# HyeonwooNoh/VQA-Transfer-ExternalData

Measured on AMD Instinct MI355X. Metric: VQA train samples/sec (img+question) at bs512, higher is better.
Workload: dtype f32

## Files before the change

include/vqa_hot.h:

```cpp
#ifndef VQA_HOT_H
#define VQA_HOT_H

#include <stdint.h>

#ifdef __cplusplus
extern "C" {
#endif

#define VQA_HOT_ABI_VERSION 5

enum {
    VQA_OK = 0,
    VQA_ERR_ARG = -1,
    VQA_ERR_ALIGN = -2,
    VQA_ERR_LAUNCH = -3,
    VQA_ERR_UNSUPPORTED = -4,
    VQA_ERR_WORKSPACE = -5
};

int vqa_hot_version(void);
const char* vqa_hot_error_string(int code);

int vqa_gather_features(const float* table, const int32_t* nbox_table, const int64_t* idx,
                        float* V, int32_t* nb, int B, int R, int D, int64_t N, void* stream);
// ... 145 lines not shown
int vqa_vtail_supported(int rep, int R, int H, int D);
int vqa_vtail_set_mode(int mode);
int vqa_attn_pool_bwd_ds(const float* dpooled, const float* V, const float* att, float* ds, float* part_db, int B, int rep,
                         int R, int H, int D, void* stream);
int vqa_attn_pool_bwd_ds_v16(const float* dpooled, const uint16_t* V, const float* att, float* ds, float* part_db, int B,
                             int rep, int R, int H, int D, void* stream);
int vqa_ln_relu_att_bwd(const float* ds, const float* qv, const float* w, const uint8_t* keep_att, float keep_prob,
                        const float* pre, const float* mean, const float* rstd, const float* gamma, const float* beta,
                        float* dpre, float* part_dgamma, float* part_dbeta, float* part_dbias, float* dqv, float* part_dw,
                        int B, int rep, int R, int H, int D, void* stream);
int64_t vqa_colsum_vtail_workspace_floats(int M, int N);
int vqa_colsum_vtail(const float* X0, const float* X1, const float* X2, const float* X3, const float* Xb, int M, int N,
                     float* out0, float* out1, float* out2, float* out3, float* outb, float* workspace,
                     int64_t workspace_floats, void* stream);

enum {
    VQA_STAT_LOSS_TRAIN = 0, VQA_STAT_LOSS_REPORT, VQA_STAT_ALL_SCORE, VQA_STAT_EXIST_SCORE,
    VQA_STAT_TEST_SCORE, VQA_STAT_TEST_OBJ_SCORE, VQA_STAT_TEST_ATTR_SCORE, VQA_STAT_TRAIN_EXIST_SCORE,
    VQA_STAT_MAX_EXIST, VQA_STAT_MAX_TRAIN_EXIST, VQA_STAT_TEST_OBJ_MAX, VQA_STAT_TEST_ATTR_MAX,
    VQA_STAT_TEST_MAX, VQA_STAT_TEST_MAX_EXIST, VQA_STAT_MAX_TRAIN, VQA_STAT_COUNT = 16
};
int vqa_loss_fwd(const float* z, const float* target, const float* train_mask, const float* obj_mask,
                 const float* attr_mask, const float* exist_mask, int use_train_mask_in_loss, float inv_batch,
                 float* stats, int32_t* pred, float* dz, int B, int A, void* stream);
int vqa_loss2_fwd(const float* z_fixed, const float* z_tuned, const float* target, const float* train_mask,
                  const float* obj_mask, const float* attr_mask, const float* exist_mask, float inv_batch, float* stats,
                  int32_t* pred, float* dz_fixed, float* dz_tuned, float* z_sum, int sum_mode, int B, int A, void* stream);
int vqa_rowmin_mask_fwd(const float* z, const float* exist_mask, float* z_masked, float* rowmin, int B, int A, void* stream);
int vqa_rowmin_mask_bwd(float* dz, const float* z, const float* rowmin, const float* exist_mask, int B, int A, void* stream);
int vqa_softmax_ce_fwd(const float* z, const int32_t* label, const float* valid, int topk,
// ... 36 lines not shown
                                 const float* bias, uint64_t seed, uint64_t offset, float keep_prob, float* att, float* pooled,
                                 int B, int rep, int R, int H, int D, void* stream);
int vqa_attn_pool_bwd_rep_seeded(const float* dpooled, const float* v, const float* qv, const float* V, const float* att,
                                 const float* w, uint64_t seed, uint64_t offset, float keep_prob, float* dv, float* dqv,
                                 float* part_dw, float* part_db, int B, int rep, int R, int H, int D, void* stream);
int vqa_ln_act_fwd_seeded(const float* pre, const float* gamma, const float* beta, uint64_t seed, uint64_t offset,
                          float keep_prob, float* y, float* mean, float* rstd, int G, int rows, int N, int act, void* stream);
int vqa_ln_act_bwd_seeded(const float* dy, const float* pre, const float* mean, const float* rstd, const float* gamma,
                          const float* beta, uint64_t seed, uint64_t offset, float keep_prob, float* dpre,
                          float* part_dgamma, float* part_dbeta, float* part_dbias, int G, int rows, int N, int act,
                          void* stream);
int vqa_ln_relu_att_bwd_seeded(const float* ds, const float* qv, const float* w, uint64_t seed, uint64_t offset,
                               float keep_prob, const float* pre, const float* mean, const float* rstd, const float* gamma,
                               const float* beta, float* dpre, float* part_dgamma, float* part_dbeta, float* part_dbias,
                               float* dqv, float* part_dw, int B, int rep, int R, int H, int D, void* stream);

typedef struct {
    int32_t B, R, D, H, T, W, A, Vq;
    int64_t N_img;
    int32_t model_type;
    float keep_att;
    float keep_joint;
    float inv_global_batch;
    int32_t flags;
    int32_t num_marginal;
    int32_t ent_cols;
    float extra_weight;
    int32_t map_dim;
    int32_t La;
} vqa_dims_t;
// ... 74 lines not shown
    int32_t keep_seeded;
} vqa_batch_t;
#define VQA_KEEP_SITE_ATT 1
#define VQA_KEEP_SITE_JOINT 2
#define VQA_KEEP_SITE_JOINT2 4
#define VQA_KEEP_SITE_TILE 8
#define VQA_KEEP_SITE_WORD 16

int64_t vqa_fusion_workspace_bytes(const vqa_dims_t* dims);
int vqa_fusion_tensor(const vqa_dims_t* dims, const char* name, int64_t* offset_bytes, int64_t* n_elems);
int vqa_fusion_forward(const vqa_dims_t* dims, const vqa_params_t* params, const vqa_batch_t* batch,
                       void* workspace, int64_t workspace_bytes, int want_dz, void* stream);
int vqa_fusion_backward(const vqa_dims_t* dims, const vqa_params_t* params, const vqa_params_t* grads,
                        const vqa_batch_t* batch, void* workspace, int64_t workspace_bytes,
                        float* embed_slice_sq, void* stream);

typedef struct {
    int32_t B, n, R, D, H, W, A, Vq, n_ws;
    int32_t L;
    int32_t flags;
    float keep_att, keep_joint;
    float global_valid[2];
} vqa_pretrain_dims_t;

typedef struct { float *w, *b, *beta[4], *gamma[4]; } vqa_pt_fc_t;

typedef struct {
    float* wordset_map;
    float* l_glove;
    vqa_pt_fc_t spat_v_linear_v;
// ... 302 lines not shown
```

vqa-transfer-externaldata_amd/_lib.py:

```python
from __future__ import annotations

import ctypes as C
import os

_HERE = os.path.dirname(os.path.abspath(__file__))
_LIB_PATH = os.path.join(_HERE, "libvqahot.so")


class VqaHotError(RuntimeError):
    pass


def lib_path():
    return _LIB_PATH


class Dims(C.Structure):
    _fields_ = [("B", C.c_int32), ("R", C.c_int32), ("D", C.c_int32), ("H", C.c_int32), ("T", C.c_int32),
                ("W", C.c_int32), ("A", C.c_int32), ("Vq", C.c_int32), ("N_img", C.c_int64),
                ("model_type", C.c_int32), ("keep_att", C.c_float), ("keep_joint", C.c_float),
                ("inv_global_batch", C.c_float), ("flags", C.c_int32),
                ("num_marginal", C.c_int32), ("ent_cols", C.c_int32), ("extra_weight", C.c_float),
                ("map_dim", C.c_int32), ("La", C.c_int32)]

# ... 212 lines not shown
    "vqa_attn_pool_fwd_rep": (_I, [_P, _P, _P, _P, _P, _P, _P, _F, _P, _P, _I, _I, _I, _I, _I, _P]),
    "vqa_attn_pool_bwd_rep": (_I, [_P, _P, _P, _P, _P, _P, _P, _F, _P, _P, _P, _P, _I, _I, _I, _I, _I, _P]),
    "vqa_vtail_supported": (_I, [_I, _I, _I, _I]),
    "vqa_vtail_set_mode": (_I, [_I]),
    "vqa_gru_h0skip_set_mode": (_I, [_I]),
    "vqa_attn_pool_bwd_ds": (_I, [_P, _P, _P, _P, _P, _I, _I, _I, _I, _I, _P]),
    "vqa_attn_pool_bwd_ds_v16": (_I, [_P, _P, _P, _P, _P, _I, _I, _I, _I, _I, _P]),
    "vqa_ln_relu_att_bwd": (_I, [_P, _P, _P, _P, _F] + [_P] * 11 + [_I, _I, _I, _I, _I, _P]),
    "vqa_attn_pool_fwd_seeded": (_I, [_P, _P, _P, _I, _P, _P, _P, _U, _U, _F, _P, _P, _I, _I, _I, _I, _I, _P]),
    "vqa_attn_pool_bwd_seeded": (_I, [_P, _P, _P, _P, _I, _P, _P, _U, _U, _F, _P, _P, _P, _P, _I, _I, _I, _I, _I, _P]),
    "vqa_attn_pool_fwd_rep_seeded": (_I, [_P, _P, _P, _P, _P, _P, _U, _U, _F, _P, _P, _I, _I, _I, _I, _I, _P]),
    "vqa_attn_pool_bwd_rep_seeded": (_I, [_P, _P, _P, _P, _P, _P, _U, _U, _F, _P, _P, _P, _P, _I, _I, _I, _I, _I, _P]),
    "vqa_ln_act_fwd_seeded": (_I, [_P, _P, _P, _U, _U, _F, _P, _P, _P, _I, _I, _I, _I, _P]),
    "vqa_ln_act_bwd_seeded": (_I, [_P, _P, _P, _P, _P, _P, _U, _U, _F, _P, _P, _P, _P, _I, _I, _I, _I, _P]),
    "vqa_ln_relu_att_bwd_seeded": (_I, [_P, _P, _P, _U, _U, _F] + [_P] * 11 + [_I, _I, _I, _I, _I, _P]),
    "vqa_colsum_vtail_workspace_floats": (_L, [_I, _I]),
    "vqa_colsum_vtail": (_I, [_P] * 5 + [_I, _I] + [_P] * 6 + [_L, _P]),
    "vqa_loss_fwd": (_I, [_P, _P, _P, _P, _P, _P, _I, _F, _P, _P, _P, _I, _I, _P]),
    "vqa_loss2_fwd": (_I, [_P, _P, _P, _P, _P, _P, _P, _F, _P, _P, _P, _P, _P, _I, _I, _I, _P]),
    "vqa_rowmin_mask_fwd": (_I, [_P, _P, _P, _P, _I, _I, _P]),
    "vqa_rowmin_mask_bwd": (_I, [_P, _P, _P, _P, _I, _I, _P]),
    "vqa_report_reduce": (_I, [_P, _I, _P, _P]),
    "vqa_report_key": (C.c_char_p, [_I]),
    "vqa_sumsq": (_I, [_P, _L, _P, _P, _P, _L, _P]),
    "vqa_sumsq_workspace_floats": (_L, [_L]),
    "vqa_clip_adam": (_I, [_P, _P, _P, _P, _L, _P, _F, _F, _F, _F, _F, _P]),
    "vqa_dropout_mask": (_I, [_P, _L, C.c_uint64, C.c_uint64, _F, _P]),
    "vqa_clip_adam_dev": (_I, [_P, _P, _P, _P, _L, _P, _F, _P, _F, _F, _F, _P]),
    "vqa_embed2_fwd": (_I, [_P, _P, _P, _P, _I, _I, _I, _I, _P]),
    "vqa_embed2_bwd": (_I, [_P, _P, _P, _P, _I, _I, _I, _I, _P]),
# ... 139 lines not shown
```

vqa-transfer-externaldata_amd/csrc/attention.hip:

```cpp
#include "keep_launch.h"

namespace {

constexpr int MAX_R = 1024;

typedef float f32x4v __attribute__((ext_vector_type(4)));
typedef unsigned u32x2v __attribute__((ext_vector_type(2)));

template <typename VT> struct VMem;
template <> struct VMem<float> {
    typedef f32x4v Raw;
    static __device__ __forceinline__ Raw load(const float* __restrict__ p, int64_t i4) { return reinterpret_cast<const f32x4v*>(p)[i4]; }
    static __device__ __forceinline__ f32x4v widen(Raw r) { return r; }
    static __device__ __forceinline__ float4 load_f4(const float* __restrict__ p, int64_t i4) { return reinterpret_cast<const float4*>(p)[i4]; }
};
template <> struct VMem<uint16_t> {
    typedef u32x2v Raw;
    static __device__ __forceinline__ Raw load(const uint16_t* __restrict__ p, int64_t i4) { return reinterpret_cast<const u32x2v*>(p)[i4]; }
    static __device__ __forceinline__ f32x4v widen(Raw r) {
        f32x4v x;
        x.x = __uint_as_float(r.x << 16); x.y = __uint_as_float(r.x & 0xFFFF0000u);
        x.z = __uint_as_float(r.y << 16); x.w = __uint_as_float(r.y & 0xFFFF0000u);
        return x;
    }
// ... 119 lines not shown
        for (int k = 0; k < H4L; ++k) {
            const f32x4v q = qw4[lane + 64 * k];
            if (KP != KEEP_NONE) {
                const unsigned mm = m[i][k];
                acc += (x[i][k].x * q.x * (float)(mm & 0xFFu) + x[i][k].y * q.y * (float)((mm >> 8) & 0xFFu) +
                        x[i][k].z * q.z * (float)((mm >> 16) & 0xFFu) + x[i][k].w * q.w * (float)(mm >> 24)) * inv_keep;
            } else {
                acc += x[i][k].x * q.x + x[i][k].y * q.y + x[i][k].z * q.z + x[i][k].w * q.w;
            }
        }
        acc = wave_sum(acc);
        if (lane == 0 && row0 + 8 * i < R) s[row0 + 8 * i] = acc + bias0;
    }
}

template <int H4L, int D4T, int KP, typename VT = float, typename... KS>
__global__ __launch_bounds__(FWD_THREADS, 4) void attn_pool_fwd_fast_kernel(
    const float* __restrict__ v, const float* __restrict__ qv, const VT* __restrict__ V,
    const int32_t* __restrict__ nb, const float* __restrict__ w, const float* __restrict__ bias,
    const uint8_t* __restrict__ keepmask, float inv_keep, float* __restrict__ att_out, float* __restrict__ pooled, int R,
    int rep, KS... ks) {
    constexpr int H = H4L * 256, D = D4T * 2048, D4 = D / 4;
    extern __shared__ __attribute__((aligned(16))) float lds[];
    float* qw = lds;
    float* s = lds + H;
    const int b = blockIdx.x, lane = threadIdx.x & 63, wave = threadIdx.x >> 6;
    const int mem = b / rep;
    const f32x4v* vb4 = reinterpret_cast<const f32x4v*>(v + (int64_t)mem * R * H);
    const unsigned* mb4 = KP == KEEP_BYTES ? reinterpret_cast<const unsigned*>(keepmask + (int64_t)b * R * H) : nullptr;
    const VT* Vb = V + (int64_t)mem * R * D;

    typename VMem<VT>::Raw xv[FAST_PF][D4T];
#pragma unroll
    for (int j = 0; j < FAST_PF; ++j)
#pragma unroll
        for (int c = 0; c < D4T; ++c) xv[j][c] = VMem<VT>::load(Vb, (int64_t)min(j, R - 1) * D4 + threadIdx.x + c * FWD_THREADS);

    for (int h = threadIdx.x; h < H; h += FWD_THREADS) qw[h] = qv[(int64_t)b * H + h] * w[h];
    const float bias0 = bias[0];

    const f32x4v* qw4 = reinterpret_cast<const f32x4v*>(qw);
    if constexpr (KP == KEEP_SEEDED) {
        KeepSeed sq = keep_seed_of(ks...);
        sq.word0 += (uint64_t)b * R * (H / 4);
        attn_score_rows<H4L, 3, KP>(vb4, mb4, qw4, s, R, wave, inv_keep, bias0, lane, true, sq);
        attn_score_rows<H4L, 2, KP>(vb4, mb4, qw4, s, R, wave + 24, inv_keep, bias0, lane, false, sq);
    } else {
        attn_score_rows<H4L, 3, KP>(vb4, mb4, qw4, s, R, wave, inv_keep, bias0, lane, true);
        attn_score_rows<H4L, 2, KP>(vb4, mb4, qw4, s, R, wave + 24, inv_keep, bias0, lane, false);
    }
    __syncthreads();

    if (wave == 0) {
        const int n_valid = nb[mem];
        float mx = -INFINITY;
        for (int r = lane; r < R; r += 64) {
            const float x = (r < n_valid) ? s[r] : -INFINITY;
// ... 821 lines not shown
    VQA_CHECK_LAUNCH();
    return VQA_OK;
}

extern "C" int vqa_attn_pool_bwd_ds_v16(const float* dpooled, const uint16_t* V, const float* att, float* ds, float* part_db,
                                        int B, int rep, int R, int H, int D, void* stream) {
    VQA_REQUIRE(dpooled && V && att && ds && part_db && B >= 0, VQA_ERR_ARG);
    VQA_REQUIRE(vqa_vtail_supported(rep, R, H, D), VQA_ERR_UNSUPPORTED);
    VQA_REQUIRE(vqa_aligned16(dpooled) && v_aligned(V), VQA_ERR_ALIGN);
    if (B == 0) return VQA_OK;
    hipLaunchKernelGGL(attn_pool_bwd_ds_kernel<uint16_t>, dim3(B), dim3(BWD_THREADS), 0, (hipStream_t)stream, dpooled, V, att,
                       ds, part_db, R);
    VQA_CHECK_LAUNCH();
    return VQA_OK;
}
```

vqa-transfer-externaldata_amd/csrc/fusion_model.hip:

```cpp
#include <stdlib.h>
#include <string.h>

#include <string>
#include <vector>

#include "keep_launch.h"

namespace {

struct Entry { const char* name; int64_t off; int64_t n; int esz; };

struct Layout {
    std::vector<Entry> e;
    int64_t total = 0;
    int64_t add(const char* name, int64_t n, int esz = 4) {
        const int64_t off = total;
        e.push_back({name, off, n, esz});
        total += ((n * esz + 255) / 256) * 256;
        return off;
    }
    const Entry* find(const char* name) const {
        for (const auto& x : e)
            if (strcmp(x.name, name) == 0) return &x;
        return nullptr;
// ... 167 lines not shown

inline bool env_on(const char* name, bool dflt) {
    const char* e = getenv(name);
    return e == nullptr ? dflt : atoi(e) != 0;
}
inline bool xcat_enabled() { static const bool v = env_on("VQA_HOT_XCAT", true); return v; }
inline bool repack_enabled() { static const bool v = env_on("VQA_HOT_REPACK", false); return v; }
inline bool gru_ws_on() { static const bool v = env_on("VQA_HOT_GRU_WS", true); return v; }
inline bool visual_late_enabled() { static const bool v = env_on("VQA_HOT_VISUAL_LATE", true); return v; }
inline bool ln_pair_enabled() { static const bool v = env_on("VQA_HOT_LN_PAIR", true); return v; }
int g_vtail_mode = -1;
inline int vtail_mode() {
    if (g_vtail_mode < 0) g_vtail_mode = env_on("VQA_HOT_VTAIL", true) ? 1 : 0;
    return g_vtail_mode;
}
int g_h0skip_mode = -1;
inline int h0skip_mode() {
    if (g_h0skip_mode < 0) {
        const char* e = getenv("VQA_HOT_GRU_H0SKIP");
        g_h0skip_mode = e == nullptr ? 1 : (atoi(e) & 3);
    }
    return g_h0skip_mode;
}
int side_max_blocks() {
    static int v = -1;
    if (v < 0) {
        const char* e = getenv("VQA_HOT_SIDE_BLOCKS");
        v = e ? atoi(e) : 0;
    }
    return v;
// ... 381 lines not shown
        if (n_elems) *n_elems = (int64_t)dims->B * dims->H;
        return VQA_OK;
    }
    const Entry* e = L.find(key);
    if (e == nullptr) return VQA_ERR_ARG;
    if (offset_bytes) *offset_bytes = e->off;
    if (n_elems) *n_elems = e->n;
    return VQA_OK;
}

extern "C" int vqa_vtail_set_mode(int mode) {
    g_vtail_mode = mode < 0 ? -1 : (mode ? 1 : 0);
    return vtail_mode();
}

extern "C" int vqa_gru_h0skip_set_mode(int mode) {
    g_h0skip_mode = mode < 0 ? -1 : (mode & 3);
    return h0skip_mode();
}

namespace {

struct Step {
    const vqa_dims_t& d;
    const vqa_params_t* const P;
    const vqa_params_t* const G;
    const vqa_batch_t* const bt;
    const Layout L;
    const Ctx c;
    const int mt;
// ... 43 lines not shown
    const bool ws_ok = gru_ws_on() && (live_rows == nullptr || (T > 0 && live_rows[T - 1] > 0));
    if (ws_ok && (dir == GRU_FWD ? vqa_gru_ws_supported((int)T, (int)B, (int)H) : vqa_gru_ws_bwd_supported((int)T, (int)B, (int)H)) == 1)
        return GRU_WS;
    return live_rows != nullptr ? GRU_LIVE : GRU_CHAINS;
}


void fwd_visual_plan(Step& s) {
    s.sd = &side_stream();
    s.forked = fork_side(s.c, *s.sd);
    s.fuse_gather = !(s.d.flags & VQA_FLAG_BF16_GEMM) && gather_mode(&s.d) == 1 && (s.D % 32 == 0) && (s.H % 4 == 0) &&
                    vqa_aligned16(s.bt->table);
    s.visual_late = !s.forked && visual_late_enabled();
}

int fwd_visual(const Step& s) {
    const Ctx cv = s.side_ctx();
    const vqa_params_t* P = s.P;
    const vqa_batch_t* bt = s.bt;
    const int64_t B = s.B, R = s.R, D = s.D, H = s.H;
    {
        ProbeScope ps("gather", cv.st);
        if (feat16(s.d))
            TRY(vqa_gather_features_bf16(reinterpret_cast<const uint16_t*>(bt->table), bt->nbox_table, bt->image_idx,
                                         cv.u16("V_ft"), cv.i32("num_V_ft"), (int)B, (int)R, (int)D, s.d.N_img, cv.st));
        else
            TRY(vqa_gather_features(bt->table, bt->nbox_table, bt->image_idx, s.fuse_gather ? nullptr : cv.f("V_ft"),
                                    cv.i32("num_V_ft"), (int)B, (int)R, (int)D, s.d.N_img, cv.st));
    }
    if (s.fuse_gather) {
        {
            ProbeScope ps("v_linear_v.fwd_gemm", cv.st);
            TRY(vqa_gemm_f32_gather((int)(B * R), (int)H, (int)D, bt->table, (int)D, bt->image_idx, (int)R, s.d.N_img,
                                    P->v_linear_v.w, (int)H, cv.f("pre_v"), (int)H, P->v_linear_v.b, cv.f("V_ft"), (int)D,
                                    cv.st));
        }
        ProbeScope ps("v_linear_v.ln_fwd", cv.st);
        TRY(vqa_ln_relu_fwd(cv.f("pre_v"), P->v_linear_v.gamma, P->v_linear_v.beta, nullptr, 1.f, cv.f("v_linear_v"),
                            cv.f("mean_v"), cv.f("rstd_v"), (int)B, (int)R, (int)H, cv.st));
    } else {
        TRY(fc_ln_relu_fwd(cv, cv.f("V_ft"), B * R, D, H, P->v_linear_v, (int)R, "pre_v", "v_linear_v", "mean_v", "rstd_v",
                           NO_KEEP, 1.f));
    }
    if (s.mt == VQA_MODEL_ADAPT) {
        VQA_REQUIRE(P->v_adapt.w != nullptr && P->v_adapt.gamma != nullptr, VQA_ERR_ARG);
        TRY(fc_ln_relu_fwd(cv, cv.f("V_ft"), B * R, D, H, P->v_adapt, (int)R, "pre_va", "v_adapt", "mean_va", "rstd_va",
                           NO_KEEP, 1.f));
    }
    return VQA_OK;
}

int fwd_question(Step& s) {
    const Ctx& c = s.c;
    const vqa_params_t* P = s.P;
    const vqa_batch_t* bt = s.bt;
    const int64_t B = s.B, H = s.H, T = s.T, W = s.W, Wp = s.Wp;
    if (s.mt == VQA_MODEL_BI) {
        TRY(bi_question_fwd(c, P, bt));
// ... 72 lines not shown
                                (int)B, (int)H, c.st));
            s.lin_in = c.f("q_L_mean_noise");
        }
    }
    return VQA_OK;
}

int fwd_q_linear_v(const Step& s) {
    return fc_ln_relu_fwd(s.c, s.qv_in, s.B, s.H, s.H, s.P->q_linear_v, 1, "pre_qv", "q_linear_v", "mean_qv", "rstd_qv", NO_KEEP, 1.f);
}

int fwd_attention(const Step& s) {
    const Ctx& c = s.c;
    ProbeScope ps("attn_pool.fwd", c.st);
    const bool v16 = feat16(s.d);
    const void* V = v16 ? (const void*)c.u16("V_ft") : (const void*)c.f(s.mt == VQA_MODEL_ADAPT ? "v_adapt" : "V_ft");
    return vqa_attn_fwd_run(c.f("v_linear_v"), c.f("q_linear_v"), V, v16, c.i32("num_V_ft"), s.P->score.w, s.P->score.b,
                            keep_site(s.bt, VQA_KEEP_SITE_ATT).src(s.d.keep_att, s.H), c.f("att_score"), c.f("pooled_V_ft"),
                            (int)s.B, 1, (int)s.R, (int)s.H, (int)s.Dp, c.st);
}

int fwd_linear_l(Step& s) {
    const Ctx& c = s.c;
    const vqa_params_t* P = s.P;
    const int64_t B = s.B, H = s.H, Dp = s.Dp;
    s.pair = ln_pair_ok(s.d, P);
    if (!s.pair) {
        TRY(fc_ln_relu_fwd(c, c.f("pooled_V_ft"), B, Dp, H, P->pooled_linear_l, 1, "pre_pl", "pooled_linear_l", "mean_pl",
                           "rstd_pl", NO_KEEP, 1.f));
        return fc_ln_relu_fwd(c, s.lin_in, B, H, H, P->q_linear_l, 1, "pre_ll", "l_linear_l", "mean_ll", "rstd_ll", NO_KEEP, 1.f);
// ... 108 lines not shown
    fwd_visual_plan(s);
    if (!s.visual_late) TRY(fwd_visual(s));
    TRY(side_record(s));
    TRY(fwd_question(s));
    TRY(fwd_question_code(s));
    TRY(fwd_q_linear_v(s));
    TRY(side_wait(s));
    if (s.visual_late) TRY(fwd_visual(s));
    TRY(fwd_attention(s));
    TRY(fwd_linear_l(s));
    TRY(fwd_joint(s));
    TRY(fwd_head(s));
    return fwd_loss(s, want_dz);
}

extern "C" int vqa_fusion_backward(const vqa_dims_t* dims, const vqa_params_t* P, const vqa_params_t* G,
                                   const vqa_batch_t* bt, void* workspace, int64_t workspace_bytes,
                                   float* embed_slice_sq, void* stream) {
    return vqa_fusion_backward_phases(dims, P, G, bt, workspace, workspace_bytes, embed_slice_sq, 15, stream);
}

namespace {


int bwd_head(const Step& s) {
    const Ctx& c = s.c;
    const vqa_params_t* P = s.P;
    const vqa_params_t* G = s.G;
    const int64_t B = s.B, H = s.H, W = s.W, A = s.A;
    ProbeScope ps_head("head.bwd_gemm", c.st);
// ... 172 lines not shown
                                         (int)R, (int)H, (int)D, c.st));
        }
        {
            ProbeScope ps("v_linear_v.ln_bwd", c.st);
            TRY(vqa_ln_relu_att_bwd_run(c.f("ds"), c.f("q_linear_v"), P->score.w, keep_site(bt, VQA_KEEP_SITE_ATT).src(s.d.keep_att, H),
                                        c.f("pre_v"), c.f("mean_v"), c.f("rstd_v"), P->v_linear_v.gamma, P->v_linear_v.beta,
                                        c.f("d_pre_v"), c.part(0), c.part(1), c.part(2), c.f("d_qv"), c.f("part_dw"), (int)B, 1, (int)R,
                                        (int)H, (int)D, c.st));
            TRY(vqa_colsum_vtail(c.part(0), c.part(1), c.part(2), c.f("part_dw"), c.f("part_db"), (int)B, (int)H,
                                 G->v_linear_v.gamma, G->v_linear_v.beta, G->v_linear_v.b, G->score.w, G->score.b, c.colsum_ws(),
                                 c.colsum_ws_floats(), c.st));
        }
        ProbeScope ps("v_linear_v.dw_gemm", c.st);
        return gemm_x(c, 1, D, H, B * R, c.f("V_ft"), (int)D, c.f("d_pre_v"), (int)H, G->v_linear_v.w, (int)H);
    }
    {
        ProbeScope ps("attn_pool.bwd", c.st);
        const bool v16 = feat16(s.d);
        const void* V = v16 ? (const void*)c.u16("V_ft") : (const void*)c.f(s.mt == VQA_MODEL_ADAPT ? "v_adapt" : "V_ft");
        TRY(vqa_attn_bwd_run(c.f("d_pooled"), c.f("v_linear_v"), c.f("q_linear_v"), V, v16, c.f("att_score"), P->score.w,
                             keep_site(bt, VQA_KEEP_SITE_ATT).src(s.d.keep_att, H), c.f("d_v"), c.f("d_qv"), c.f("part_dw"),
                             c.f("part_db"), (int)B, 1, (int)R, (int)H, (int)Dp, c.st));
    }
    if (s.mt == VQA_MODEL_ADAPT) {
        TRY(vqa_outer_rows(c.f("att_score"), c.f("d_pooled"), c.f("d_va"), (int)B, (int)R, (int)H, c.st));
        TRY(fc_ln_relu_bwd(c, c.f("d_va"), c.f("V_ft"), B * R, D, H, P->v_adapt, &G->v_adapt, (int)R, "pre_va", "mean_va",
                           "rstd_va", NO_KEEP, 1.f, "d_pre_va", nullptr, false));
    }
    if (G->score.w != nullptr) {
        ProbeScope ps("attn_pool.bwd", c.st);
// ... 167 lines not shown
```

vqa-transfer-externaldata_amd/csrc/keep_launch.h:

```cpp
#pragma once
#include "vqa_common.h"

int vqa_ln_act_fwd_run(const float* pre, const float* gamma, const float* beta, const KeepSrc& keep, float* y, float* mean,
                       float* rstd, int G, int rows, int N, int act, void* stream);
int vqa_ln_act_bwd_run(const float* dy, const float* pre, const float* mean, const float* rstd, const float* gamma,
                       const float* beta, const KeepSrc& keep, float* dpre, float* part_dgamma, float* part_dbeta,
                       float* part_dbias, int G, int rows, int N, int act, void* stream);
int vqa_ln_relu_att_bwd_run(const float* ds, const float* qv, const float* w, const KeepSrc& keep, const float* pre,
                            const float* mean, const float* rstd, const float* gamma, const float* beta, float* dpre,
                            float* part_dgamma, float* part_dbeta, float* part_dbias, float* dqv, float* part_dw, int B, int rep,
                            int R, int H, int D, void* stream);

int vqa_attn_fwd_run(const float* v, const float* qv, const void* V, bool v_bf16, const int32_t* nb, const float* w,
                     const float* bias, const KeepSrc& keep, float* att, float* pooled, int B, int rep, int R, int H, int D,
                     void* stream, bool seeded_one_query = false);
int vqa_attn_bwd_run(const float* dpooled, const float* v, const float* qv, const void* V, bool v_bf16, const float* att,
                     const float* w, const KeepSrc& keep, float* dv, float* dqv, float* part_dw, float* part_db, int B, int rep,
                     int R, int H, int D, void* stream, bool seeded_one_query = false);
```

vqa-transfer-externaldata_amd/csrc/layernorm.hip:

```cpp
#include "keep_launch.h"

namespace {

constexpr float LN_EPS = 1e-12f;

template <int U>
struct Vec;
template <>
struct Vec<4> {
    float v[4];
    __device__ __forceinline__ void load(const float* p) {
        const float4 t = *reinterpret_cast<const float4*>(p);
        v[0] = t.x; v[1] = t.y; v[2] = t.z; v[3] = t.w;
    }
    __device__ __forceinline__ void store(float* p) const {
        *reinterpret_cast<float4*>(p) = make_float4(v[0], v[1], v[2], v[3]);
    }
    __device__ __forceinline__ void load_mask(const uint8_t* p) {
        const uchar4 t = *reinterpret_cast<const uchar4*>(p);
        v[0] = t.x; v[1] = t.y; v[2] = t.z; v[3] = t.w;
    }
    __device__ __forceinline__ void set_mask(unsigned w) {
        const uchar4 t = keep_uchar4(w);
        v[0] = t.x; v[1] = t.y; v[2] = t.z; v[3] = t.w;
// ... 437 lines not shown
    const float m2 = block_sum(s2, red) * invL;
    f32x4v* o4 = reinterpret_cast<f32x4v*>(dpre) + base4;
    float cbias[4] = {0.f, 0.f, 0.f, 0.f};
#pragma unroll
    for (int i = 0; i < RPT; ++i) {
        f32x4v o;
#pragma unroll
        for (int j = 0; j < 4; ++j) {
            const float dp = mul_rounded(rstd, d[i][j] - m1 - x[i][j] * m2);
            o[j] = dp;
            cbias[j] += dp;
        }
        o4[(ry + REG_RY * i) * N4 + cx] = o;
    }
    col_reduce_store<4>(buf0, cbias, part_dbias + (int64_t)g * N, cx, N4, cx, ry, REG_CUT, REG_RY);
}

int g_ln_reg = 1;

inline int reg_mode(int U, int rows, int N) {
    if (!g_ln_reg || U != 4) return 0;
    if (N == REG_CUT * 4 && rows == REG_RY * 9) return 1;
    if (N == REG_CUT * 4 && rows >= 2 && rows <= REG_RY * 2) return 2;
    if (N == REG_CUT * 8 && rows >= 2 && rows <= REG_RY * 2) return 3;
    return 0;
}

template <int RM>
struct RegForm {
    static constexpr int RPT = RM == 1 ? 9 : 2, CPT = RM == 3 ? 2 : 1;
// ... 370 lines not shown
                                   const float* pre, const float* mean, const float* rstd, const float* gamma,
                                   const float* beta, float* dpre, float* part_dgamma, float* part_dbeta, float* part_dbias,
                                   float* dqv, float* part_dw, int B, int rep, int R, int H, int D, void* stream) {
    return vqa_ln_relu_att_bwd_run(ds, qv, w, KeepSrc::bytes(keep_att, keep_prob), pre, mean, rstd, gamma, beta, dpre, part_dgamma,
                                   part_dbeta, part_dbias, dqv, part_dw, B, rep, R, H, D, stream);
}

extern "C" int vqa_ln_relu_att_bwd_seeded(const float* ds, const float* qv, const float* w, uint64_t seed, uint64_t offset,
                                          float keep_prob, const float* pre, const float* mean, const float* rstd,
                                          const float* gamma, const float* beta, float* dpre, float* part_dgamma,
                                          float* part_dbeta, float* part_dbias, float* dqv, float* part_dw, int B, int rep,
                                          int R, int H, int D, void* stream) {
    return vqa_ln_relu_att_bwd_run(ds, qv, w, KeepSrc::seeded(seed, offset, H, keep_prob), pre, mean, rstd, gamma, beta, dpre,
                                   part_dgamma, part_dbeta, part_dbias, dqv, part_dw, B, rep, R, H, D, stream);
}
```

vqa-transfer-externaldata_amd/fusion.py:

```python
from __future__ import annotations

import collections
import ctypes as C

import numpy as np
import torch

from . import _lib
from .engine_core import ADAM_B1, ADAM_B2, ADAM_EPS, EngineCore, carve, phase_schedule

CLIP_NORM = 20.0

FROZEN_TOP_SCOPES_VLMAP = ("q_linear_l", "pooled_linear_l", "joint_fc", "WordWeightAnswer")
TRANSFER_TOP_SCOPES_VLMAP = ("q_linear_l", "pooled_linear_l", "joint_fc")

_INT_TENSORS = {"num_V_ft", "pred"}


STANDARD_FAMILY = ("standard", "standard_word2vec", "standard_testmask")
NOC_FAMILY = ("vlmap_answer_noc", "vlmap_answer_nocarch")
FROZEN_TOP_SCOPES_NOC = ("q_linear_l", "pooled_linear_l", "joint_v", "joint_l", "WordWeightAnswerV", "WordWeightAnswerL")
TRANSFER_TOP_SCOPES_NOC = ("q_linear_l", "pooled_linear_l", "joint_v", "joint_l")
TWO_HEAD_FAMILY = ("vlmap_answer_vqa_all", "vlmap_answer_vqa_all2")
ABLATION_FAMILY = ("vlmap_answer2", "vlmap_answer_no_noise", "vlmap_answer_adapt", "vlmap_answer_full", "vlmap_answer_ent")
# ... 329 lines not shown
        self.drop_graphs()
        d.B, d.T = B, T
        d.inv_global_batch = 1.0 / float(global_batch or B)
        self._grow_workspace()
        for a in ["_" + k.name for k in KEEP_SITES] + ["_noise", "_keep_lay"]:
            if hasattr(self, a):
                delattr(self, a)

    def _grow_workspace(self):
        self._ensure_workspace(self.lib.vqa_fusion_workspace_bytes, self.dims, "vqa_fusion_workspace_bytes rejected the dims",
                               before_grow=self.drop_graphs)
        self._tensor_cache = {}
        self._reset_recurrence_word()

    def tensor(self, name):
        if name in self._tensor_cache:
            return self._tensor_cache[name]
        off, n = C.c_int64(), C.c_int64()
        _lib.check(self.lib.vqa_fusion_tensor(C.byref(self.dims), name.encode(), C.byref(off), C.byref(n)),
                   "vqa_fusion_tensor(%s)" % name)
        if name == "V_ft" and self.features == "bf16":
            t = self.workspace[off.value:off.value + 2 * n.value].view(torch.bfloat16)
            self._tensor_cache[name] = t
            return t
        raw = self.workspace[off.value:off.value + 4 * n.value]
        t = raw.view(torch.int32 if name in _INT_TENSORS else torch.float32)
        self._tensor_cache[name] = t
        return t

    def bind_inputs(self, *, table, nbox_table, answer_masks):
# ... 281 lines not shown
```

vqa-transfer-externaldata_amd/ops.py:

```python
from __future__ import annotations

import ctypes as C

import numpy as np
import torch

from . import _lib


def _p(t):
    return C.c_void_p(t.data_ptr()) if t is not None else None


def _st(t):
    return C.c_void_p(torch.cuda.current_stream(t.device).cuda_stream)


def _f32(*shape, like):
    return torch.empty(*shape, dtype=torch.float32, device=like.device)


def gemm(A, B, transA=False, transB=False, bias=None, addend=None, split_k=0, out=None):
    lib = _lib.load()
    assert A.dtype == torch.float32 and B.dtype == torch.float32 and A.stride(-1) == 1 and B.stride(-1) == 1
# ... 198 lines not shown
               "vqa_attn_pool_bwd_ds")
    return ds, pdb


def ln_relu_att_bwd(ds, qv, w, pre, mean, rstd, gamma, beta, keepmask=None, keep_prob=1.0, keep_seed=None):
    B, R, H = pre.shape
    dpre = torch.empty_like(pre)
    pg, pb, pbias, dqv, pdw = (_f32(B, H, like=pre) for _ in range(5))
    sd = _seeded(keepmask, keep_seed)
    _call("vqa_ln_relu_att_bwd_seeded" if sd else "vqa_ln_relu_att_bwd", _p(ds), _p(qv), _p(w), *(sd or (_p(keepmask),)), keep_prob,
          _p(pre), _p(mean), _p(rstd), _p(gamma), _p(beta), _p(dpre), _p(pg), _p(pb), _p(pbias), _p(dqv), _p(pdw), B, 1, R, H, 2048,
          _st(pre))
    return dpre, (pg, pb, pbias), dqv, pdw


def colsum_vtail(X0, X1, X2, X3, Xb):
    lib = _lib.load()
    M, N = X0.shape
    outs = [_f32(N, like=X0) for _ in range(4)] + [_f32(1, like=X0)]
    ws = _f32(max(int(lib.vqa_colsum_vtail_workspace_floats(M, N)), 4), like=X0)
    _lib.check(lib.vqa_colsum_vtail(_p(X0), _p(X1), _p(X2), _p(X3), _p(Xb), M, N, *[_p(o) for o in outs], _p(ws),
                                    ws.numel(), _st(X0)), "vqa_colsum_vtail")
    return outs


def loss_fwd(z, target, masks, use_train_mask=True, inv_batch=None, want_dz=True):
    lib = _lib.load()
    B, A = z.shape
    stats = _f32(B, 16, like=z)
    pred = torch.empty(B, dtype=torch.int32, device=z.device)
# ... 198 lines not shown
```

Baseline: 164,200.

## Fuse visual LayerNorm-ReLU with attention scoring and defer v_linear_v materialization

Adds a kernel that computes the visual LayerNorm+ReLU and immediately dots it with qv*w (with dropout) to produce the raw attention scores, without writing v_linear_v in the forward pass. The attention-pool forward then only runs softmax and pooling from the precomputed scores. v_linear_v is recomputed in backward (and on demand when Python reads it) only when needed. This saves a full B*R*H write plus read in the forward pass, at the cost of an extra LN recompute pass in backward and more code paths gated by an env mode.

```diff
diff --git a/include/vqa_hot.h b/include/vqa_hot.h
--- a/include/vqa_hot.h
+++ b/include/vqa_hot.h
@@ -183,6 +183,15 @@
                      float* out0, float* out1, float* out2, float* out3, float* outb, float* workspace,
                      int64_t workspace_floats, void* stream);
 
+int vqa_ln_relu_att_fwd(const float* pre, const float* gamma, const float* beta, const float* qv, const float* w,
+                        const float* bias, const uint8_t* keep_att, float keep_prob, float* y, float* mean, float* rstd,
+                        float* s_raw, int B, int rep, int R, int H, int D, void* stream);
+int vqa_attn_pool_fwd_scored(const float* V, const int32_t* nb, float* att, float* pooled, int B, int rep, int R, int H,
+                             int D, void* stream);
+int vqa_attn_pool_fwd_scored_v16(const uint16_t* V, const int32_t* nb, float* att, float* pooled, int B, int rep, int R,
+                                 int H, int D, void* stream);
+int vqa_vfwd_set_mode(int mode);
+
 enum {
     VQA_STAT_LOSS_TRAIN = 0, VQA_STAT_LOSS_REPORT, VQA_STAT_ALL_SCORE, VQA_STAT_EXIST_SCORE,
     VQA_STAT_TEST_SCORE, VQA_STAT_TEST_OBJ_SCORE, VQA_STAT_TEST_ATTR_SCORE, VQA_STAT_TRAIN_EXIST_SCORE,
@@ -249,6 +258,9 @@
                                float keep_prob, const float* pre, const float* mean, const float* rstd, const float* gamma,
                                const float* beta, float* dpre, float* part_dgamma, float* part_dbeta, float* part_dbias,
                                float* dqv, float* part_dw, int B, int rep, int R, int H, int D, void* stream);
+int vqa_ln_relu_att_fwd_seeded(const float* pre, const float* gamma, const float* beta, const float* qv, const float* w,
+                               const float* bias, uint64_t seed, uint64_t offset, float keep_prob, float* y, float* mean,
+                               float* rstd, float* s_raw, int B, int rep, int R, int H, int D, void* stream);
 
 typedef struct {
     int32_t B, R, D, H, T, W, A, Vq;
@@ -353,6 +365,8 @@
 int vqa_fusion_backward(const vqa_dims_t* dims, const vqa_params_t* params, const vqa_params_t* grads,
                         const vqa_batch_t* batch, void* workspace, int64_t workspace_bytes,
                         float* embed_slice_sq, void* stream);
+int vqa_fusion_refresh_tensor(const vqa_dims_t* dims, const vqa_params_t* params, const vqa_batch_t* batch, void* workspace,
+                              int64_t workspace_bytes, const char* name, void* stream);
 
 typedef struct {
     int32_t B, n, R, D, H, W, A, Vq, n_ws;
diff --git a/vqa-transfer-externaldata_amd/_lib.py b/vqa-transfer-externaldata_amd/_lib.py
--- a/vqa-transfer-externaldata_amd/_lib.py
+++ b/vqa-transfer-externaldata_amd/_lib.py
@@ -250,6 +250,12 @@
     "vqa_ln_act_fwd_seeded": (_I, [_P, _P, _P, _U, _U, _F, _P, _P, _P, _I, _I, _I, _I, _P]),
     "vqa_ln_act_bwd_seeded": (_I, [_P, _P, _P, _P, _P, _P, _U, _U, _F, _P, _P, _P, _P, _I, _I, _I, _I, _P]),
     "vqa_ln_relu_att_bwd_seeded": (_I, [_P, _P, _P, _U, _U, _F] + [_P] * 11 + [_I, _I, _I, _I, _I, _P]),
+    "vqa_ln_relu_att_fwd": (_I, [_P] * 7 + [_F] + [_P] * 4 + [_I, _I, _I, _I, _I, _P]),
+    "vqa_ln_relu_att_fwd_seeded": (_I, [_P] * 6 + [_U, _U, _F] + [_P] * 4 + [_I, _I, _I, _I, _I, _P]),
+    "vqa_attn_pool_fwd_scored": (_I, [_P, _P, _P, _P, _I, _I, _I, _I, _I, _P]),
+    "vqa_attn_pool_fwd_scored_v16": (_I, [_P, _P, _P, _P, _I, _I, _I, _I, _I, _P]),
+    "vqa_vfwd_set_mode": (_I, [_I]),
+    "vqa_fusion_refresh_tensor": (_I, [C.POINTER(Dims), C.POINTER(Params), C.POINTER(Batch), _P, _L, C.c_char_p, _P]),
     "vqa_colsum_vtail_workspace_floats": (_L, [_I, _I]),
     "vqa_colsum_vtail": (_I, [_P] * 5 + [_I, _I] + [_P] * 6 + [_L, _P]),
     "vqa_loss_fwd": (_I, [_P, _P, _P, _P, _P, _P, _I, _F, _P, _P, _P, _I, _I, _P]),
diff --git a/vqa-transfer-externaldata_amd/csrc/attention.hip b/vqa-transfer-externaldata_amd/csrc/attention.hip
--- a/vqa-transfer-externaldata_amd/csrc/attention.hip
+++ b/vqa-transfer-externaldata_amd/csrc/attention.hip
@@ -157,6 +157,7 @@
     }
 }
 
+constexpr int SCORES_GIVEN = 3;
 template <int H4L, int D4T, int KP, typename VT = float, typename... KS>
 __global__ __launch_bounds__(FWD_THREADS, 4) void attn_pool_fwd_fast_kernel(
     const float* __restrict__ v, const float* __restrict__ qv, const VT* __restrict__ V,
@@ -166,7 +167,7 @@
     constexpr int H = H4L * 256, D = D4T * 2048, D4 = D / 4;
     extern __shared__ __attribute__((aligned(16))) float lds[];
     float* qw = lds;
-    float* s = lds + H;
+    float* s = lds + (KP == SCORES_GIVEN ? 0 : H);
     const int b = blockIdx.x, lane = threadIdx.x & 63, wave = threadIdx.x >> 6;
     const int mem = b / rep;
     const f32x4v* vb4 = reinterpret_cast<const f32x4v*>(v + (int64_t)mem * R * H);
@@ -179,11 +180,14 @@
 #pragma unroll
         for (int c = 0; c < D4T; ++c) xv[j][c] = VMem<VT>::load(Vb, (int64_t)min(j, R - 1) * D4 + threadIdx.x + c * FWD_THREADS);
 
-    for (int h = threadIdx.x; h < H; h += FWD_THREADS) qw[h] = qv[(int64_t)b * H + h] * w[h];
-    const float bias0 = bias[0];
+    if constexpr (KP != SCORES_GIVEN)
+        for (int h = threadIdx.x; h < H; h += FWD_THREADS) qw[h] = qv[(int64_t)b * H + h] * w[h];
+    const float bias0 = KP == SCORES_GIVEN ? 0.f : bias[0];
 
     const f32x4v* qw4 = reinterpret_cast<const f32x4v*>(qw);
-    if constexpr (KP == KEEP_SEEDED) {
+    if constexpr (KP == SCORES_GIVEN) {
+        if ((int)threadIdx.x < R) s[threadIdx.x] = att_out[(int64_t)b * R + threadIdx.x];
+    } else if constexpr (KP == KEEP_SEEDED) {
         KeepSeed sq = keep_seed_of(ks...);
         sq.word0 += (uint64_t)b * R * (H / 4);
         attn_score_rows<H4L, 3, KP>(vb4, mb4, qw4, s, R, wave, inv_keep, bias0, lane, true, sq);
@@ -1035,3 +1039,26 @@
     VQA_CHECK_LAUNCH();
     return VQA_OK;
 }
+
+template <typename VT>
+static int attn_fwd_scored(const VT* V, const int32_t* nb, float* att, float* pooled, int B, int rep, int R, int H, int D,
+                           void* stream) {
+    VQA_REQUIRE(V && nb && att && pooled && B >= 0, VQA_ERR_ARG);
+    VQA_REQUIRE(vqa_vtail_supported(rep, R, H, D), VQA_ERR_UNSUPPORTED);
+    VQA_REQUIRE(v_aligned(V) && vqa_aligned16(pooled), VQA_ERR_ALIGN);
+    if (B == 0) return VQA_OK;
+    hipLaunchKernelGGL((attn_pool_fwd_fast_kernel<4, 1, SCORES_GIVEN, VT>), dim3(B), dim3(FWD_THREADS), (size_t)R * sizeof(float),
+                       (hipStream_t)stream, nullptr, nullptr, V, nb, nullptr, nullptr, nullptr, 1.f, att, pooled, R, 1);
+    VQA_CHECK_LAUNCH();
+    return VQA_OK;
+}
+
+extern "C" int vqa_attn_pool_fwd_scored(const float* V, const int32_t* nb, float* att, float* pooled, int B, int rep, int R,
+                                        int H, int D, void* stream) {
+    return attn_fwd_scored(V, nb, att, pooled, B, rep, R, H, D, stream);
+}
+
+extern "C" int vqa_attn_pool_fwd_scored_v16(const uint16_t* V, const int32_t* nb, float* att, float* pooled, int B, int rep,
+                                            int R, int H, int D, void* stream) {
+    return attn_fwd_scored(V, nb, att, pooled, B, rep, R, H, D, stream);
+}
diff --git a/vqa-transfer-externaldata_amd/csrc/fusion_model.hip b/vqa-transfer-externaldata_amd/csrc/fusion_model.hip
--- a/vqa-transfer-externaldata_amd/csrc/fusion_model.hip
+++ b/vqa-transfer-externaldata_amd/csrc/fusion_model.hip
@@ -205,6 +205,11 @@
     if (g_vtail_mode < 0) g_vtail_mode = env_on("VQA_HOT_VTAIL", true) ? 1 : 0;
     return g_vtail_mode;
 }
+int g_vfwd_mode = -1;
+inline int vfwd_mode() {
+    if (g_vfwd_mode < 0) g_vfwd_mode = env_on("VQA_HOT_VFWD", true) ? 1 : 0;
+    return g_vfwd_mode;
+}
 int g_h0skip_mode = -1;
 inline int h0skip_mode() {
     if (g_h0skip_mode < 0) {
@@ -616,6 +621,11 @@
     return vtail_mode();
 }
 
+extern "C" int vqa_vfwd_set_mode(int mode) {
+    g_vfwd_mode = mode < 0 ? -1 : (mode ? 1 : 0);
+    return vfwd_mode();
+}
+
 extern "C" int vqa_gru_h0skip_set_mode(int mode) {
     g_h0skip_mode = mode < 0 ? -1 : (mode & 3);
     return h0skip_mode();
@@ -689,6 +699,30 @@
     s.visual_late = !s.forked && visual_late_enabled();
 }
 
+bool vfwd_ok(const Step& s) {
+    const vqa_params_t* P = s.P;
+    const KeepSrc keep = keep_site(s.bt, VQA_KEEP_SITE_ATT).src(s.d.keep_att, s.H);
+    return vfwd_mode() != 0 && !side_stream().ok && visual_late_enabled() && s.mt != VQA_MODEL_ADAPT &&
+           vqa_vtail_supported(1, (int)s.R, (int)s.H, (int)s.Dp) == 1 && P->v_linear_v.gamma != nullptr &&
+           P->v_linear_v.beta != nullptr && P->score.w != nullptr && P->score.b != nullptr && vqa_aligned16(P->v_linear_v.gamma) &&
+           vqa_aligned16(P->v_linear_v.beta) && vqa_aligned16(P->score.w) && keep.err == VQA_OK && keep.words_ok();
+}
+
+int v_linear_v_store(const Step& s, const Ctx& cv) {
+    ProbeScope ps("v_linear_v.ln_fwd", cv.st);
+    return vqa_ln_act_fwd_run(cv.f("pre_v"), s.P->v_linear_v.gamma, s.P->v_linear_v.beta, KeepSrc(), cv.f("v_linear_v"),
+                              cv.f("mean_v"), cv.f("rstd_v"), (int)s.B, (int)s.R, (int)s.H, 0, cv.st);
+}
+
+int fwd_v_linear_v_ln(const Step& s, const Ctx& cv) {
+    if (!vfwd_ok(s)) return v_linear_v_store(s, cv);
+    ProbeScope ps("v_linear_v.ln_fwd", cv.st);
+    return vqa_ln_relu_att_fwd_run(cv.f("pre_v"), s.P->v_linear_v.gamma, s.P->v_linear_v.beta, cv.f("q_linear_v"), s.P->score.w,
+                                   s.P->score.b, keep_site(s.bt, VQA_KEEP_SITE_ATT).src(s.d.keep_att, s.H), nullptr,
+                                   cv.f("mean_v"), cv.f("rstd_v"), cv.f("att_score"), (int)s.B, 1, (int)s.R, (int)s.H, (int)s.Dp,
+                                   cv.st);
+}
+
 int fwd_visual(const Step& s) {
     const Ctx cv = s.side_ctx();
     const vqa_params_t* P = s.P;
@@ -703,20 +737,16 @@
             TRY(vqa_gather_features(bt->table, bt->nbox_table, bt->image_idx, s.fuse_gather ? nullptr : cv.f("V_ft"),
                                     cv.i32("num_V_ft"), (int)B, (int)R, (int)D, s.d.N_img, cv.st));
     }
-    if (s.fuse_gather) {
-        {
-            ProbeScope ps("v_linear_v.fwd_gemm", cv.st);
+    {
+        ProbeScope ps("v_linear_v.fwd_gemm", cv.st);
+        if (s.fuse_gather)
             TRY(vqa_gemm_f32_gather((int)(B * R), (int)H, (int)D, bt->table, (int)D, bt->image_idx, (int)R, s.d.N_img,
                                     P->v_linear_v.w, (int)H, cv.f("pre_v"), (int)H, P->v_linear_v.b, cv.f("V_ft"), (int)D,
                                     cv.st));
-        }
-        ProbeScope ps("v_linear_v.ln_fwd", cv.st);
-        TRY(vqa_ln_relu_fwd(cv.f("pre_v"), P->v_linear_v.gamma, P->v_linear_v.beta, nullptr, 1.f, cv.f("v_linear_v"),
-                            cv.f("mean_v"), cv.f("rstd_v"), (int)B, (int)R, (int)H, cv.st));
-    } else {
-        TRY(fc_ln_relu_fwd(cv, cv.f("V_ft"), B * R, D, H, P->v_linear_v, (int)R, "pre_v", "v_linear_v", "mean_v", "rstd_v",
-                           NO_KEEP, 1.f));
-    }
+        else
+            TRY(gemm_x(cv, 0, B * R, H, D, cv.f("V_ft"), (int)D, P->v_linear_v.w, (int)H, cv.f("pre_v"), (int)H, P->v_linear_v.b));
+    }
+    TRY(fwd_v_linear_v_ln(s, cv));
     if (s.mt == VQA_MODEL_ADAPT) {
         VQA_REQUIRE(P->v_adapt.w != nullptr && P->v_adapt.gamma != nullptr, VQA_ERR_ARG);
         TRY(fc_ln_relu_fwd(cv, cv.f("V_ft"), B * R, D, H, P->v_adapt, (int)R, "pre_va", "v_adapt", "mean_va", "rstd_va",
@@ -819,6 +849,13 @@
     const Ctx& c = s.c;
     ProbeScope ps("attn_pool.fwd", c.st);
     const bool v16 = feat16(s.d);
+    if (vfwd_ok(s)) {
+        if (v16)
+            return vqa_attn_pool_fwd_scored_v16(c.u16("V_ft"), c.i32("num_V_ft"), c.f("att_score"), c.f("pooled_V_ft"), (int)s.B, 1,
+                                                (int)s.R, (int)s.H, (int)s.Dp, c.st);
+        return vqa_attn_pool_fwd_scored(c.f("V_ft"), c.i32("num_V_ft"), c.f("att_score"), c.f("pooled_V_ft"), (int)s.B, 1, (int)s.R,
+                                        (int)s.H, (int)s.Dp, c.st);
+    }
     const void* V = v16 ? (const void*)c.u16("V_ft") : (const void*)c.f(s.mt == VQA_MODEL_ADAPT ? "v_adapt" : "V_ft");
     return vqa_attn_fwd_run(c.f("v_linear_v"), c.f("q_linear_v"), V, v16, c.i32("num_V_ft"), s.P->score.w, s.P->score.b,
                             keep_site(s.bt, VQA_KEEP_SITE_ATT).src(s.d.keep_att, s.H), c.f("att_score"), c.f("pooled_V_ft"),
@@ -957,6 +994,16 @@
     return fwd_loss(s, want_dz);
 }
 
+extern "C" int vqa_fusion_refresh_tensor(const vqa_dims_t* dims, const vqa_params_t* P, const vqa_batch_t* bt, void* workspace,
+                                         int64_t workspace_bytes, const char* name, void* stream) {
+    VQA_REQUIRE(dims_ok(dims) && P && bt && workspace && name, VQA_ERR_ARG);
+    if (strcmp(name, "v_linear_v") != 0 || dims->model_type == VQA_MODEL_LEGACY_VQA) return VQA_OK;
+    Step s(dims, P, nullptr, bt, workspace, stream);
+    VQA_REQUIRE(workspace_bytes >= s.L.total, VQA_ERR_WORKSPACE);
+    VQA_REQUIRE(vqa_aligned16(workspace), VQA_ERR_ALIGN);
+    return vfwd_ok(s) ? v_linear_v_store(s, s.c) : VQA_OK;
+}
+
 extern "C" int vqa_fusion_backward(const vqa_dims_t* dims, const vqa_params_t* P, const vqa_params_t* G,
                                    const vqa_batch_t* bt, void* workspace, int64_t workspace_bytes,
                                    float* embed_slice_sq, void* stream) {
@@ -1159,6 +1206,7 @@
         ProbeScope ps("v_linear_v.dw_gemm", c.st);
         return gemm_x(c, 1, D, H, B * R, c.f("V_ft"), (int)D, c.f("d_pre_v"), (int)H, G->v_linear_v.w, (int)H);
     }
+    if (vfwd_ok(s)) TRY(v_linear_v_store(s, c));
     {
         ProbeScope ps("attn_pool.bwd", c.st);
         const bool v16 = feat16(s.d);
diff --git a/vqa-transfer-externaldata_amd/csrc/keep_launch.h b/vqa-transfer-externaldata_amd/csrc/keep_launch.h
--- a/vqa-transfer-externaldata_amd/csrc/keep_launch.h
+++ b/vqa-transfer-externaldata_amd/csrc/keep_launch.h
@@ -10,6 +10,9 @@
                             const float* mean, const float* rstd, const float* gamma, const float* beta, float* dpre,
                             float* part_dgamma, float* part_dbeta, float* part_dbias, float* dqv, float* part_dw, int B, int rep,
                             int R, int H, int D, void* stream);
+int vqa_ln_relu_att_fwd_run(const float* pre, const float* gamma, const float* beta, const float* qv, const float* w,
+                            const float* bias, const KeepSrc& keep, float* y, float* mean, float* rstd, float* s_raw, int B,
+                            int rep, int R, int H, int D, void* stream);
 
 int vqa_attn_fwd_run(const float* v, const float* qv, const void* V, bool v_bf16, const int32_t* nb, const float* w,
                      const float* bias, const KeepSrc& keep, float* att, float* pooled, int B, int rep, int R, int H, int D,
diff --git a/vqa-transfer-externaldata_amd/csrc/layernorm.hip b/vqa-transfer-externaldata_amd/csrc/layernorm.hip
--- a/vqa-transfer-externaldata_amd/csrc/layernorm.hip
+++ b/vqa-transfer-externaldata_amd/csrc/layernorm.hip
@@ -475,6 +475,91 @@
         o4[(ry + REG_RY * i) * N4 + cx] = o;
     }
     col_reduce_store<4>(buf0, cbias, part_dbias + (int64_t)g * N, cx, N4, cx, ry, REG_CUT, REG_RY);
+}
+
+constexpr size_t ATT_FWD_LDS = (size_t)REG_RY * 9 * REG_CUT * sizeof(float);
+template <int KP, typename... KS>
+__global__ __launch_bounds__(REG_CUT * REG_RY) void ln_att_fwd_reg_kernel(
+    const float* __restrict__ pre, const float* __restrict__ gamma, const float* __restrict__ beta,
+    const float* __restrict__ qv, const float* __restrict__ w, const float* __restrict__ bias,
+    const uint8_t* __restrict__ keep_att, float inv_keep, float* __restrict__ y, float* __restrict__ mean_out,
+    float* __restrict__ rstd_out, float* __restrict__ s_raw, int rpt, KS... ks) {
+#pragma clang fp contract(off)
+    constexpr int RPT = 9, N4 = REG_CUT, N = N4 * 4, ROWS = REG_RY * RPT;
+    extern __shared__ __attribute__((aligned(16))) float term[];
+    __shared__ float red[16];
+    const int g = blockIdx.x, cx = threadIdx.x % REG_CUT, ry = __builtin_amdgcn_readfirstlane(threadIdx.x / REG_CUT);
+    const int64_t base4 = (int64_t)g * ROWS * N4;
+    const f32x4v* p4 = reinterpret_cast<const f32x4v*>(pre) + base4;
+    const unsigned* m4 = KP == KEEP_BYTES ? reinterpret_cast<const unsigned*>(keep_att) + base4 : nullptr;
+    const float invL = 1.f / ((float)ROWS * (float)N);
+    f32x4v x[RPT];
+    unsigned km[RPT];
+#pragma unroll
+    for (int i = 0; i < RPT; ++i) {
+        const int o = (ry + REG_RY * i) * N4 + cx;
+        x[i] = p4[o];
+        if (KP == KEEP_BYTES) km[i] = m4[o];
+    }
+    float xs = 0.f;
+#pragma unroll
+    for (int i = 0; i < RPT; ++i) { xs += x[i].x; xs += x[i].y; xs += x[i].z; xs += x[i].w; }
+    const float xsum = block_sum(xs, red);
+    float q = 0.f;
+#pragma unroll
+    for (int i = 0; i < RPT; ++i) {
+#pragma unroll
+        for (int j = 0; j < 4; ++j) x[i][j] = __builtin_fmaf(-xsum, invL, x[i][j]);
+        if (i == 0) q = __builtin_fmaf(x[0].x, x[0].x, x[0].y * x[0].y);
+        else { q = __builtin_fmaf(x[i].x, x[i].x, q); q = __builtin_fmaf(x[i].y, x[i].y, q); }
+        q = __builtin_fmaf(x[i].z, x[i].z, q);
+        q = __builtin_fmaf(x[i].w, x[i].w, q);
+    }
+    const float rstd = 1.f / sqrtf(__builtin_fmaf(invL, block_sum(q, red), LN_EPS));
+    if (threadIdx.x == 0) { mean_out[g] = invL * xsum; rstd_out[g] = rstd; }
+    const f32x4v ga = reinterpret_cast<const f32x4v*>(gamma)[cx];
+    const f32x4v be = reinterpret_cast<const f32x4v*>(beta)[cx];
+    const f32x4v qw = reinterpret_cast<const f32x4v*>(qv + (int64_t)g * N)[cx] * reinterpret_cast<const f32x4v*>(w)[cx];
+    f32x4v* y4 = y != nullptr ? reinterpret_cast<f32x4v*>(y) + base4 : nullptr;
+#pragma unroll
+    for (int i = 0; i < RPT; ++i) {
+        if (i < rpt) {
+            const int o = (ry + REG_RY * i) * N4 + cx;
+            f32x4v v;
+#pragma unroll
+            for (int j = 0; j < 4; ++j) v[j] = fmaxf(__builtin_fmaf(ga[j], rstd * x[i][j], be[j]), 0.f);
+            if (y4 != nullptr) y4[o] = v;
+            float t;
+            if (KP == KEEP_NONE) {
+                t = __builtin_fmaf(v.w, qw.w, __builtin_fmaf(v.z, qw.z, __builtin_fmaf(v.x, qw.x, v.y * qw.y)));
+            } else {
+                unsigned mm = km[i];
+                if constexpr (KP == KEEP_SEEDED) {
+                    const KeepSeed sd = keep_seed_of(ks...);
+                    mm = keep_word4(sd.key, sd.word0 + (uint64_t)(base4 + o), sd.thr);
+                }
+                const f32x4v p = v * qw;
+                t = __builtin_fmaf(p.w, (float)(mm >> 24),
+                                   __builtin_fmaf(p.z, (float)((mm >> 16) & 0xFFu),
+                                                  __builtin_fmaf(p.x, (float)(mm & 0xFFu), p.y * (float)((mm >> 8) & 0xFFu))));
+            }
+            term[o] = t;
+        }
+    }
+    __syncthreads();
+    const int lane = threadIdx.x & 63, wave = __builtin_amdgcn_readfirstlane(threadIdx.x >> 6);
+    const float bias0 = bias[0];
+    for (int r = wave; r < ROWS; r += REG_CUT * REG_RY / 64) {
+        float acc = 0.f;
+#pragma unroll
+        for (int k = 0; k < 4; ++k) {
+            const float t = term[r * N4 + lane + 64 * k];
+            if (KP == KEEP_NONE) acc += t;
+            else acc = __builtin_fmaf(inv_keep, t, acc);
+        }
+        acc = wave_sum(acc);
+        if (lane == 0) s_raw[(int64_t)g * ROWS + r] = acc + bias0;
+    }
 }
 
 int g_ln_reg = 1;
@@ -875,3 +960,39 @@
     return vqa_ln_relu_att_bwd_run(ds, qv, w, KeepSrc::seeded(seed, offset, H, keep_prob), pre, mean, rstd, gamma, beta, dpre,
                                    part_dgamma, part_dbeta, part_dbias, dqv, part_dw, B, rep, R, H, D, stream);
 }
+
+int vqa_ln_relu_att_fwd_run(const float* pre, const float* gamma, const float* beta, const float* qv, const float* w,
+                            const float* bias, const KeepSrc& keep, float* y, float* mean, float* rstd, float* s_raw, int B,
+                            int rep, int R, int H, int D, void* stream) {
+    VQA_REQUIRE(pre && gamma && beta && qv && w && bias && mean && rstd && s_raw, VQA_ERR_ARG);
+    VQA_REQUIRE(keep.err == VQA_OK, keep.err);
+    VQA_REQUIRE(B >= 0, VQA_ERR_ARG);
+    VQA_REQUIRE(vqa_vtail_supported(rep, R, H, D), VQA_ERR_UNSUPPORTED);
+    VQA_REQUIRE(vqa_aligned16(pre) && vqa_aligned16(gamma) && vqa_aligned16(beta) && vqa_aligned16(qv) && vqa_aligned16(w) &&
+                    vqa_aligned16(y) && keep.words_ok(),
+                VQA_ERR_ALIGN);
+    if (B == 0) return VQA_OK;
+    hipStream_t st = (hipStream_t)stream;
+    keep_dispatch(keep, [&](auto kp, auto... ks) {
+        hipLaunchKernelGGL((ln_att_fwd_reg_kernel<decltype(kp)::value, decltype(ks)...>), dim3(B), dim3(REG_CUT * REG_RY),
+                           ATT_FWD_LDS, st, pre, gamma, beta, qv, w, bias, keep.mask, keep.inv_keep(), y, mean, rstd, s_raw, 9,
+                           ks...);
+    });
+    VQA_CHECK_LAUNCH();
+    return VQA_OK;
+}
+
+extern "C" int vqa_ln_relu_att_fwd(const float* pre, const float* gamma, const float* beta, const float* qv, const float* w,
+                                   const float* bias, const uint8_t* keep_att, float keep_prob, float* y, float* mean,
+                                   float* rstd, float* s_raw, int B, int rep, int R, int H, int D, void* stream) {
+    return vqa_ln_relu_att_fwd_run(pre, gamma, beta, qv, w, bias, KeepSrc::bytes(keep_att, keep_prob), y, mean, rstd, s_raw, B, rep,
+                                   R, H, D, stream);
+}
+
+extern "C" int vqa_ln_relu_att_fwd_seeded(const float* pre, const float* gamma, const float* beta, const float* qv,
+                                          const float* w, const float* bias, uint64_t seed, uint64_t offset, float keep_prob,
+                                          float* y, float* mean, float* rstd, float* s_raw, int B, int rep, int R, int H, int D,
+                                          void* stream) {
+    return vqa_ln_relu_att_fwd_run(pre, gamma, beta, qv, w, bias, KeepSrc::seeded(seed, offset, H, keep_prob), y, mean, rstd, s_raw,
+                                   B, rep, R, H, D, stream);
+}
diff --git a/vqa-transfer-externaldata_amd/fusion.py b/vqa-transfer-externaldata_amd/fusion.py
--- a/vqa-transfer-externaldata_amd/fusion.py
+++ b/vqa-transfer-externaldata_amd/fusion.py
@@ -367,6 +367,10 @@
         self._reset_recurrence_word()
 
     def tensor(self, name):
+        if name == "v_linear_v" and getattr(self, "_bs", None) is not None:
+            _lib.check(self.lib.vqa_fusion_refresh_tensor(C.byref(self.dims), C.byref(self._p_struct), C.byref(self._bs),
+                                                          C.c_void_p(self.workspace.data_ptr()), self.workspace.numel(),
+                                                          name.encode(), self._stream()), "vqa_fusion_refresh_tensor")
         if name in self._tensor_cache:
             return self._tensor_cache[name]
         off, n = C.c_int64(), C.c_int64()
diff --git a/vqa-transfer-externaldata_amd/ops.py b/vqa-transfer-externaldata_amd/ops.py
--- a/vqa-transfer-externaldata_amd/ops.py
+++ b/vqa-transfer-externaldata_amd/ops.py
@@ -236,6 +236,24 @@
     return dpre, (pg, pb, pbias), dqv, pdw
 
 
+def ln_relu_att_fwd(pre, gamma, beta, qv, w, bias, keepmask=None, keep_prob=1.0, keep_seed=None, want_y=False):
+    B, R, H = pre.shape
+    y = torch.empty_like(pre) if want_y else None
+    mean, rstd, s_raw = _f32(B, like=pre), _f32(B, like=pre), _f32(B, R, like=pre)
+    sd = _seeded(keepmask, keep_seed)
+    _call("vqa_ln_relu_att_fwd_seeded" if sd else "vqa_ln_relu_att_fwd", _p(pre), _p(gamma), _p(beta), _p(qv), _p(w), _p(bias),
+          *(sd or (_p(keepmask),)), keep_prob, _p(y), _p(mean), _p(rstd), _p(s_raw), B, 1, R, H, 2048, _st(pre))
+    return s_raw, mean, rstd, y
+
+
+def attn_pool_fwd_scored(s_raw, V, nb):
+    B, R, D = V.shape
+    att, pooled = s_raw.clone(), _f32(B, D, like=s_raw)
+    _call("vqa_attn_pool_fwd_scored_v16" if V.dtype == torch.bfloat16 else "vqa_attn_pool_fwd_scored", _p(V), _p(nb), _p(att),
+          _p(pooled), B, 1, R, 1024, D, _st(V))
+    return att, pooled
+
+
 def colsum_vtail(X0, X1, X2, X3, Xb):
     lib = _lib.load()
     M, N = X0.shape
```

After: 165,400, median of 6. Within noise of the previous version (+0.7%).
